# fundamentalvision/BEVFormer

Hardware: NVIDIA H100
Metric: BEV queries/sec (bevformer_base 200x200x256, 6 cams) fwd+bwd (higher is better)
Workload: dtype bf16

## Files before the change

bevformer_b200/_lib.py:

```python
from __future__ import annotations

import ctypes
import os
import threading

from . import build as _build

_lock = threading.Lock()
_lib = None

c_void_p, c_int, c_int64 = ctypes.c_void_p, ctypes.c_int, ctypes.c_int64

SIGNATURES = {
    "bevf_version": (c_int, []),
    "bevf_last_error": (ctypes.c_char_p, []),
    "bevf_launch_count": (c_int64, []),
    "bevf_msda_forward": (c_int, [c_void_p, c_int, c_void_p, c_void_p, c_void_p, c_void_p,
                                  c_void_p, c_int] + [c_int] * 7 + [c_void_p]),
    "bevf_msda_backward": (c_int, [c_void_p, c_int, c_void_p, c_void_p, c_void_p, c_void_p,
                                   c_void_p, c_int, c_void_p, c_void_p, c_void_p] + [c_int] * 7
                           + [c_void_p]),
    "bevf_msda_rows_forward": (c_int, [c_void_p, c_int, c_void_p, c_void_p, c_void_p, c_void_p,
                                       c_void_p, c_int, c_void_p] + [c_int] * 7 + [c_void_p]),
    "bevf_msda_rows_backward": (c_int, [c_void_p, c_int, c_void_p, c_void_p, c_void_p, c_void_p,
                                        c_void_p, c_int, c_void_p, c_void_p, c_void_p, c_void_p]
                                + [c_int] * 7 + [c_void_p]),
    "bevf_msda_rows_backward_ordered": (c_int, [c_void_p, c_int, c_void_p, c_void_p, c_void_p, c_void_p,
                                                c_void_p, c_int, c_void_p, c_void_p, c_void_p, c_void_p,
                                                c_void_p] + [c_int] * 7 + [c_void_p]),
    "bevf_msda_set_backward_mode": (c_int, [c_int]),
    "bevf_abs_max": (c_int, [c_void_p, c_int, c_int64, c_void_p, c_void_p]),
    "bevf_msda_rows_backward_f16acc": (c_int, [c_void_p, c_int, c_void_p, c_void_p, c_void_p, c_void_p, c_void_p, c_int,
                                               c_void_p, c_void_p, c_void_p, c_void_p, c_void_p, c_void_p] + [c_int] * 7
                                       + [c_void_p]),
    "bevf_gv16_unscale": (c_int, [c_void_p, c_void_p, c_void_p, c_int64, c_void_p]),
    "bevf_msda_rows_backward_mixed": (c_int, [c_void_p, c_int, c_void_p, c_void_p, c_void_p, c_void_p, c_void_p, c_void_p,
                                              c_int, c_void_p, c_void_p, c_void_p, c_int, c_void_p, c_void_p, c_void_p,
                                              c_void_p] + [c_int] * 7 + [c_void_p]),
    "bevf_gv_merge": (c_int, [c_void_p, c_void_p, c_void_p, c_void_p, c_int, c_int, c_int, c_int, c_void_p]),
    "bevf_msda_fx_frac_bits": (c_int, [c_int64, c_int, c_int]),
    "bevf_msda_backward_fx": (c_int, [c_void_p, c_int, c_void_p, c_void_p, c_void_p, c_void_p, c_void_p, c_int,
                                      c_void_p, c_void_p, c_int, c_void_p, c_void_p] + [c_int] * 7 + [c_void_p]),
    "bevf_msda_rows_backward_fx": (c_int, [c_void_p, c_int, c_void_p, c_void_p, c_void_p, c_void_p, c_void_p, c_int,
                                           c_void_p, c_void_p, c_int, c_void_p, c_void_p, c_void_p] + [c_int] * 7
                                   + [c_void_p]),
    "bevf_msda_fx_convert": (c_int, [c_void_p, c_void_p, c_int, c_void_p, c_int, c_int, c_int64, c_void_p]),
    "bevf_msda_rows_backward_dense": (c_int, [c_void_p, c_int, c_void_p, c_void_p, c_void_p, c_void_p, c_void_p,
                                              c_void_p, c_int, c_void_p, c_void_p, c_void_p, c_void_p, c_void_p]
                                      + [c_int] * 7 + [c_void_p]),
    "bevf_msda_set_dense_backward": (c_int, [c_int]),
    "bevf_msda_get_dense_backward": (c_int, []),
    "bevf_msda_dense_plan": (c_int, [c_void_p, c_int, c_int, c_int, c_void_p, c_int, c_void_p]),
    "bevf_sca_plan_workspace_ints": (c_int64, [c_int, c_int]),
    "bevf_sca_plan_build": (c_int, [c_void_p] * 10 + [c_int] * 5 + [c_void_p]),
    "bevf_msda_rows_forward_staged": (c_int, [c_void_p, c_int, c_void_p, c_void_p, c_void_p, c_void_p, c_void_p,
                                              c_void_p, c_int, c_void_p] + [c_int] * 7 + [c_void_p]),
    "bevf_sca_prep_forward": (c_int, [c_void_p] * 7 + [c_int] * 8 + [c_void_p]),
    "bevf_sca_prep_backward": (c_int, [c_void_p] * 6 + [c_int] * 8 + [c_void_p]),
    "bevf_tsa_prep_forward": (c_int, [c_void_p] * 5 + [c_int] * 6 + [c_void_p]),
    "bevf_tsa_prep_backward": (c_int, [c_void_p] * 5 + [c_int] * 7 + [c_void_p]),
    "bevf_layernorm_forward": (c_int, [c_void_p] * 4 + [c_int] + [c_void_p] * 5
# ... 89 lines not shown
```

bevformer_b200/csrc/msda.cu:

```cuda
#include <cuda_fp16.h>

#include <cstdlib>
#include <cstring>
#include <type_traits>

#include "msda_common.cuh"

namespace bevf {

template <typename T, typename TO>
__global__ void __launch_bounds__(kThreads)
msda_fwd_d32(const T *__restrict__ value, const int64_t *__restrict__ level_hw,
             const int64_t *__restrict__ level_start, const float *__restrict__ loc,
             const float *__restrict__ attn, TO *__restrict__ out,
             const int *__restrict__ row_map, int S, int M, int Q, int L, int P, int magic,
             int iters, long long rows) {
    constexpr int VEC = Vec<T>::N, LANES = 32 / VEC, G = 32 / LANES;
    constexpr bool kHalf = std::is_same<T, bf16>::value;
    __shared__ LevelTab tab;
    load_level_tab(level_hw, level_start, L, M * 32, tab);

    const int lane = threadIdx.x & 31, warp = threadIdx.x >> 5;
    const int sub = lane % LANES, grp = lane / LANES;
    for (int it = 0; it < iters; ++it) {
    long long row = (((long long)blockIdx.x * (kThreads / 32) + warp) * iters + it) * G + grp;
    if (row - grp >= rows) break;
// ... 456 lines not shown

static std::atomic<int> g_bwd_mode{-1};
static int bwd_split_enabled() {
    int v = g_bwd_mode.load(std::memory_order_relaxed);
    if (v < 0) {
        const char *e = getenv("BEVF_MSDA_BWD");
        v = (e && e[0] == 's') ? 1 : 0;
        g_bwd_mode.store(v, std::memory_order_relaxed);
    }
    return v;
}
static unsigned splat_direct_mask() {
    static long v = -1;
    if (v < 0) {
        const char *e = getenv("BEVF_SPLAT_DIRECT");
        v = e ? strtol(e, nullptr, 0) : 0;
    }
    return (unsigned)v;
}

int dense_coarse_backward(const char *who, const int64_t *hw_dev, const int64_t *ls_dev, const int32_t *hw_host,
                          const float *loc, const float *attn, const void *grad_out, float *grad_value,
                          const int32_t *map_range, int NB, int S, int M, int L, int P, cudaStream_t st,
                          unsigned *handled, HostLevels *host_levels);

static cudaStream_t g_side_stream = nullptr;
constexpr int kSideEvents = 64;
static cudaEvent_t g_side_events[kSideEvents];
static std::atomic<unsigned> g_side_ev_next{0};

template <typename TG, int kM>
static int launch_splat_km(const char *who, const float *loc, const float *attn, const void *go, float *gv,
                           const int *row_map, const int *order, const int64_t *hw, const int64_t *ls,
                           int S, int M, int Q, int L, int P, long long pairs, unsigned level_mask,
                           cudaStream_t st) {
    static bool attr_done = false;
    if (!attr_done) {
        if (cudaFuncSetAttribute(msda_bwd_splat_d32<TG, kM>, cudaFuncAttributeMaxDynamicSharedMemorySize,
                                 (int)splat_smem_bytes(kSplatMaxHeads, sizeof(TG))) != cudaSuccess) {
            cudaGetLastError();
            return fail("%s: cannot reserve shared memory for the splat kernel", who);
        }
        attr_done = true;
    }
    const unsigned grid = (unsigned)((pairs + kSplatG - 1) / kSplatG);
    msda_bwd_splat_d32<TG, kM><<<grid, 32 * M, splat_smem_bytes(M, sizeof(TG)), st>>>(
        loc, attn, (const TG *)go, gv, row_map, order, hw, ls, S, M, Q, L, P, pairs, splat_direct_mask(),
// ... 60 lines not shown
        if constexpr (std::is_same<T, bf16>::value) {
            if (D != 32) return fail("%s: fp16 grad_value needs head_dim 32", who);
            constexpr int G = Vec<T>::N;
            const int iters = pick_iters(rows, G);
            const long long per_block = (long long)(kThreads / 32) * G * iters;
            const unsigned grid = (unsigned)((rows + per_block - 1) / per_block);
            msda_bwd_d32<T, TG, true, __half><<<grid, kThreads, 0, st>>>((const T *)value, hw, ls, loc, attn, (const TG *)go,
                                                                       reinterpret_cast<__half *>(gv), gl, ga, row_map, S, M,
                                                                       Q, L, P, (65536 + P - 1) / P, iters, rows, 0u, hl,
                                                                       mixed ? mixed->amax : nullptr);
            return check_launch(who);
        } else {
            return fail("%s: fp16 grad_value needs a bf16 value tensor", who);
        }
    }
    if (mixed && mixed->gv16) {
        if constexpr (std::is_same<T, bf16>::value) {
            if (D != 32) return fail("%s: mixed accumulation needs head_dim 32", who);
            constexpr int G = Vec<T>::N;
            const int iters = pick_iters(rows, G);
            const long long per_block = (long long)(kThreads / 32) * G * iters;
            const unsigned grid = (unsigned)((rows + per_block - 1) / per_block);
            msda_bwd_d32<T, TG, true><<<grid, kThreads, 0, st>>>((const T *)value, hw, ls, loc, attn, (const TG *)go, gv, gl, ga,
                                                               row_map, S, M, Q, L, P, (65536 + P - 1) / P, iters, rows, 0u,
                                                               hl, mixed->amax, mixed->gv16, mixed->mask, mixed->side_start,
                                                               mixed->S_side);
            return check_launch(who);
        } else {
            return fail("%s: mixed accumulation needs a bf16 value tensor", who);
        }
    }
    if (D == 32) {
        constexpr int G = Vec<T>::N;
        const int iters = pick_iters(rows, G);
        const long long per_block = (long long)(kThreads / 32) * G * iters;
        const unsigned grid = (unsigned)((rows + per_block - 1) / per_block);
        const int mode = done_levels ? 0 : bwd_split_enabled();
        if (mode != 0 && std::is_same<T, __half>::value)
            return fail("%s: the split / hybrid backward modes take fp32 or bf16 only (fp16 needs mode 0)", who);
        const bool can_split = M <= kSplatMaxHeads && S * (long long)M * 32 < (1ll << 31);
        if (mode == 1 && can_split) {
            if (int e = launch_splat<TG>(who, loc, attn, go, gv, row_map, order, hw, ls, S, M, Q, L, P,
                                         rows / M, 0xffffffffu, st))
                return e;
            msda_bwd_d32<T, TG, false><<<grid, kThreads, 0, st>>>((const T *)value, hw, ls, loc, attn,
                                                                  (const TG *)go, gv, gl, ga, row_map, S, M,
                                                                  Q, L, P, (65536 + P - 1) / P, iters, rows, 0u, hl);
        } else if (mode == 2 && can_split && L >= 2 && g_side_stream) {
// ... 107 lines not shown

extern "C" int bevf_msda_rows_forward(const void *value, int value_dtype, const int64_t *level_hw,
                                      const int64_t *level_start, const float *loc,
                                      const float *attn, void *out, int out_dtype,
                                      const int32_t *row_map, int B, int S, int M, int D, int R,
                                      int L, int P, void *stream) {
    if (!row_map && R > 0) return fail("%s: row_map is null", "bevf_msda_rows_forward");
    return msda_forward_impl("bevf_msda_rows_forward", value, value_dtype, level_hw, level_start,
                             loc, attn, out, out_dtype, row_map, B, S, M, D, R, L, P, stream);
}

extern "C" int bevf_msda_rows_backward(const void *value, int value_dtype, const int64_t *level_hw,
                                       const int64_t *level_start, const float *loc,
                                       const float *attn, const void *grad_out, int grad_out_dtype,
                                       float *grad_value, float *grad_loc, float *grad_attn,
                                       const int32_t *row_map, int B, int S, int M, int D, int R,
                                       int L, int P, void *stream) {
    if (!row_map && R > 0) return fail("%s: row_map is null", "bevf_msda_rows_backward");
    return msda_backward_impl("bevf_msda_rows_backward", value, value_dtype, level_hw, level_start,
                              loc, attn, grad_out, grad_out_dtype, grad_value, grad_loc, grad_attn,
                              row_map, nullptr, B, S, M, D, R, L, P, stream);
}

static std::atomic<int> g_dense_mode{-1};
static int dense_mode() {
    int v = g_dense_mode.load(std::memory_order_relaxed);
    if (v < 0) {
        const char *e = getenv("BEVF_MSDA_DENSE");
        v = e ? atoi(e) : 0;
        if (v < 0 || v > 1) v = 1;
        g_dense_mode.store(v, std::memory_order_relaxed);
    }
    return v;
}
static int ensure_side_stream(const char *who) {
    if (g_side_stream) return 0;
    if (cudaStreamCreateWithFlags(&g_side_stream, cudaStreamNonBlocking) != cudaSuccess) {
        cudaGetLastError();
        g_side_stream = nullptr;
        return fail("%s: cannot create the second stream", who);
    }
    for (int i = 0; i < kSideEvents; ++i) cudaEventCreateWithFlags(&g_side_events[i], cudaEventDisableTiming);
    return 0;
}

extern "C" int bevf_msda_set_dense_backward(int mode) {
    if (mode < 0 || mode > 2)
        return fail("%s: mode must be 0 (off), 1 (same stream) or 2 (second stream)", "bevf_msda_set_dense_backward");
    if (mode == 2)
        if (int e = ensure_side_stream("bevf_msda_set_dense_backward")) return e;
    g_dense_mode.store(mode, std::memory_order_relaxed);
    return 0;
}

extern "C" int bevf_msda_get_dense_backward(void) { return dense_mode(); }

extern "C" int bevf_msda_rows_backward_dense(const void *value, int value_dtype, const int64_t *level_hw,
                                             const int64_t *level_start, const int32_t *level_hw_host,
                                             const float *loc, const float *attn, const void *grad_out,
                                             int grad_out_dtype, float *grad_value, float *grad_loc,
                                             float *grad_attn, const int32_t *row_map, const int32_t *map_range,
                                             int B, int S, int M, int D, int R, int L, int P, void *stream) {
    const char *who = "bevf_msda_rows_backward_dense";
    if (!row_map && R > 0) return fail("%s: row_map is null", who);
    if (int e = check_dims(who, B, S, M, D, R, L, P)) return e;
    if (R == 0) return 0;
    if (!level_hw_host || !map_range || !level_hw || !level_start || !loc || !attn || !grad_out || !grad_value)
        return fail("%s: null pointer argument", who);
    cudaStream_t st = (cudaStream_t)stream;
    unsigned handled = 0;
    HostLevels hl;
    memset(&hl, 0, sizeof(hl));
    const int mode = dense_mode();
    cudaEvent_t join = nullptr;
    if (value_dtype == BEVF_DTYPE_F16 || grad_out_dtype == BEVF_DTYPE_F16)
        return fail("%s: fp32 or bf16 only (fp16 runs on bevf_msda_rows_backward)", who);
    if (mode != 0 && D == 32 && grad_out_dtype == BEVF_DTYPE_BF16 && aligned16(loc) && aligned16(attn) &&
        aligned16(grad_out) && aligned16(grad_value)) {
        cudaStream_t ds = st;
        if (mode == 2 && g_side_stream) {
            cudaEvent_t fork = g_side_events[g_side_ev_next.fetch_add(1) % kSideEvents];
            join = g_side_events[g_side_ev_next.fetch_add(1) % kSideEvents];
            cudaEventRecord(fork, st);
            cudaStreamWaitEvent(g_side_stream, fork, 0);
            ds = g_side_stream;
        }
        const int e = dense_coarse_backward(who, level_hw, level_start, level_hw_host, loc, attn, grad_out, grad_value,
                                            map_range, B, S, M, L, P, ds, &handled, &hl);
        if (join) cudaEventRecord(join, g_side_stream);
        if (e) {
            if (join) cudaStreamWaitEvent(st, join, 0);
            return e;
        }
    }
    const int e = msda_backward_impl(who, value, value_dtype, level_hw, level_start, loc, attn, grad_out,
                                     grad_out_dtype, grad_value, grad_loc, grad_attn, row_map, nullptr, B, S, M, D,
                                     R, L, P, stream, handled, &hl);
    if (join) cudaStreamWaitEvent(st, join, 0);
    return e;
}

extern "C" int bevf_msda_rows_backward_f16acc(const void *value, int value_dtype, const int64_t *level_hw,
                                              const int64_t *level_start, const float *loc, const float *attn,
                                              const void *grad_out, int grad_out_dtype, void *grad_value_f16,
                                              const uint32_t *amax_bits, float *grad_loc, float *grad_attn,
                                              const int32_t *row_map, const int32_t *group_order, int B, int S,
                                              int M, int D, int R, int L, int P, void *stream) {
    const char *who = "bevf_msda_rows_backward_f16acc";
    if (!row_map && R > 0) return fail("%s: row_map is null", who);
    if (!grad_value_f16 || !amax_bits) return fail("%s: null pointer argument", who);
    MixedGv mx;
    mx.amax = amax_bits;
    return msda_backward_impl(who, value, value_dtype, level_hw, level_start, loc, attn, grad_out, grad_out_dtype,
                              reinterpret_cast<float *>(grad_value_f16), grad_loc, grad_attn, row_map, group_order, B, S,
                              M, D, R, L, P, stream, 0u, nullptr, true, &mx);
}

extern "C" int bevf_msda_rows_backward_mixed(const void *value, int value_dtype, const int64_t *level_hw,
                                             const int64_t *level_start, const int32_t *level_hw_host,
                                             const float *loc, const float *attn, const void *grad_out,
                                             int grad_out_dtype, void *grad_value_fine_f16, float *grad_value_side,
                                             const uint32_t *amax_bits, int num_f16_levels, float *grad_loc,
                                             float *grad_attn, const int32_t *row_map, const int32_t *group_order,
                                             int B, int S, int M, int D, int R, int L, int P, void *stream) {
    const char *who = "bevf_msda_rows_backward_mixed";
    if (!row_map && R > 0) return fail("%s: row_map is null", who);
    if (!level_hw_host || !grad_value_fine_f16 || !grad_value_side || !amax_bits)
        return fail("%s: null pointer argument", who);
    if (L <= 1 || L > kMaxLevels || num_f16_levels < 1 || num_f16_levels >= L)
        return fail("%s: num_f16_levels must be in [1, L - 1]", who);
    if (value_dtype != BEVF_DTYPE_BF16 || D != 32) return fail("%s: needs a bf16 value tensor and head_dim 32", who);
    if (!aligned16(grad_value_fine_f16) || !aligned16(grad_value_side))
        return fail("%s: device pointers must be 16-byte aligned", who);
    HostLevels hl;
    memset(&hl, 0, sizeof(hl));
    long long start = 0;
    for (int l = 0; l < L; ++l) {
        const int h = level_hw_host[2 * l], w = level_hw_host[2 * l + 1];
        if (h <= 0 || w <= 0 || h >= 32768 || w >= 32768) return fail("%s: bad host level shape", who);
        hl.h[l] = h; hl.w[l] = w; hl.start[l] = (int)start;
        start += (long long)h * w;
    }
    if (start != S) return fail("%s: host level shapes do not add up to S (%lld vs %lld)", who, start, S);
    MixedGv mx;
    mx.amax = amax_bits;
    mx.gv16 = reinterpret_cast<__half *>(grad_value_fine_f16);
    mx.mask = (1u << num_f16_levels) - 1u;
    mx.side_start = hl.start[num_f16_levels];
    mx.S_side = S - mx.side_start;
    return msda_backward_impl(who, value, value_dtype, level_hw, level_start, loc, attn, grad_out, grad_out_dtype,
                              grad_value_side, grad_loc, grad_attn, row_map, group_order, B, S, M, D, R, L, P, stream, 0u,
                              &hl, false, &mx);
}

namespace bevf {
int fx_bounds_launch(const char *who, const float *attn, const void *grad_out, int grad_out_dtype,
                     const int32_t *row_map, long long qrows, int M, int D, int L, int P, uint32_t *bounds,
                     cudaStream_t st);

static int msda_backward_fx_impl(const char *who, const void *value, int value_dtype, const int64_t *level_hw,
                                 const int64_t *level_start, const float *loc, const float *attn, const void *grad_out,
                                 int grad_out_dtype, int64_t *grad_value_fx, uint32_t *bounds, int frac_bits,
                                 float *grad_loc, float *grad_attn, const int32_t *row_map, int B, int S, int M, int D,
                                 int Q, int L, int P, void *stream) {
    if (int e = check_dims(who, B, S, M, D, Q, L, P)) return e;
    const long long qrows = (row_map ? 1ll : (long long)B) * Q;
    if (qrows == 0) return 0;
    if (!bounds || !grad_value_fx || !attn || !grad_out) return fail("%s: null pointer argument", who);
    const int kmax = bevf_msda_fx_frac_bits(Q, L, P);
    if (frac_bits < 0 || frac_bits > kmax)
        return fail("%s: frac_bits must be in [0, %lld] for this launch (bevf_msda_fx_frac_bits)", who, kmax);
    cudaStream_t st = (cudaStream_t)stream;
    if (int e = fx_bounds_launch(who, attn, grad_out, grad_out_dtype, row_map, qrows, M, D, L, P, bounds, st)) return e;
    FxGv fx;
    fx.bounds = bounds;
// ... 57 lines not shown
```

bevformer_b200/csrc/msda_dense.cu:

```cuda
#include <cuda.h>

#include <cstdlib>
#include <cstring>
#include <mutex>

#include "msda_common.cuh"

namespace bevf {

constexpr int kDnK = 16;
constexpr int kDnMaxBins = 32;
constexpr int kDnBinLevels = 4;
constexpr int kDnTileBytes = 128 * kDnK * 2;
constexpr int kDnTransposeBytes = 16 * 144;

struct DenseBins {
    int nbins, L;
    int s0[kDnMaxBins], n[kDnMaxBins];
    int nlev[kDnMaxBins];
    int lev[kDnMaxBins][kDnBinLevels];
    HostLevels hl;
};

namespace dn {
// ... 60 lines not shown
    uint4 v;
    asm volatile("ld.global.nc.v4.u32 {%0, %1, %2, %3}, [%4];" : "=r"(v.x), "=r"(v.y), "=r"(v.z), "=r"(v.w) : "l"(p));
    return v;
}
__device__ __forceinline__ unsigned short lds16(uint32_t addr) {
    unsigned short h;
    asm volatile("ld.shared.u16 %0, [%1];" : "=h"(h) : "r"(addr) : "memory");
    return h;
}
__device__ __forceinline__ void sts16(uint32_t addr, unsigned short h) {
    asm volatile("st.shared.u16 [%0], %1;" ::"r"(addr), "h"(h) : "memory");
}
__device__ __forceinline__ unsigned short bf16_add(unsigned short old, float x) {
    const float v = __uint_as_float((uint32_t)old << 16) + x;
    return __bfloat16_as_ushort(__float2bfloat16_rn(v));
}
}

template <int kTiles, int P, int NT>
__global__ void __launch_bounds__(128 * NT + 256, 1)
msda_bwd_dense_tc(const __grid_constant__ DenseBins bins, const int64_t *__restrict__ level_hw,
                  const int64_t *__restrict__ level_start, const float *__restrict__ loc,
                  const float *__restrict__ attn, const bf16 *__restrict__ grad_out,
                  float *__restrict__ grad_value, const int *__restrict__ map_range, int NB, int S, int M, int L,
                  int chunk_rows, int dbg) {
    static_assert(P == 4 || P == 8, "points per level: 4 or 8");
    static_assert(kTiles == 4, "accumulator tiles per bin: 2 per issuer warpgroup");
    static_assert(NT >= 1 && NT <= 3, "scatter teams");
    constexpr int kThreadsAll = 128 * NT + 256;
    constexpr int kSlabBytes = kTiles * kDnTileBytes;
    constexpr int kMine = kTiles / 2;
    constexpr int kColsPerWarp = 32 / P;
    constexpr int kWarpsPerLevel = kDnK / kColsPerWarp;
    constexpr int kLevelsPerPass = 4 / kWarpsPerLevel;
    constexpr int kMaxPass = kDnBinLevels / kLevelsPerPass;
    extern __shared__ __align__(1024) uint8_t smem_raw[];
    uint8_t *smem = reinterpret_cast<uint8_t *>((reinterpret_cast<uintptr_t>(smem_raw) + 1023) & ~uintptr_t(1023));
    uint8_t *slab = smem;
    uint8_t *gtile = smem + NT * kSlabBytes;
    float *tr = reinterpret_cast<float *>(gtile + NT * 4096);
    uint64_t *bar_full = reinterpret_cast<uint64_t *>(reinterpret_cast<uint8_t *>(tr) + 8 * kDnTransposeBytes);
    uint64_t *bar_empty = bar_full + NT;
    uint32_t *s_dirty = reinterpret_cast<uint32_t *>(bar_empty + NT);
    __shared__ int s_h[kMaxLevels], s_w[kMaxLevels], s_start[kMaxLevels];
    __shared__ int s_bad;

    const int tid = threadIdx.x, lane = tid & 31;
    const int team = tid >> 7, tt = tid & 127, tw = tt >> 5;
// ... 242 lines not shown
                float *trw = tr + (iw * 4 + w4) * (kDnTransposeBytes / 4);
                const int sub = lane & 7;
#pragma unroll
                for (int i = 0; i < kMine; ++i) {
                    const int tile = 2 * i + iw;
                    if (!((udirty >> tile) & 1u)) continue;
#pragma unroll
                    for (int h = 0; h < 2; ++h) {
#pragma unroll
                        for (int j = 0; j < 4; ++j)
#pragma unroll
                            for (int hh = 0; hh < 2; ++hh)
                                *reinterpret_cast<float2 *>(trw + (8 * hh + (lane >> 2)) * 36 + 8 * j + 2 * (lane & 3)) =
                                    make_float2(acc[i][h][4 * j + 2 * hh], acc[i][h][4 * j + 2 * hh + 1]);
                        __syncwarp();
#pragma unroll
                        for (int q = 0; q < 4; ++q) {
                            const int rr = 4 * q + (lane >> 3);
                            const int row = tile * 128 + h * 64 + w4 * 16 + rr;
                            const float4 v = *reinterpret_cast<const float4 *>(trw + rr * 36 + sub * 4);
                            const bool nz = ((__float_as_uint(v.x) | __float_as_uint(v.y) | __float_as_uint(v.z) |
                                              __float_as_uint(v.w)) & 0x7fffffffu) != 0u;
                            if (nz && row < nb) {
                                float *gp = grad_value + (((long long)b * S + s0 + row) * M + m) * 32 + sub * 4;
                                red_add_v4(gp, v.x, v.y, v.z, v.w);
                            }
                        }
                        __syncwarp();
                    }
                }
            }
            unit_bar();
        }
    }
}

}

namespace bevf {

static long dense_env(const char *name, long dflt) {
    const char *e = getenv(name);
    return e ? strtol(e, nullptr, 0) : dflt;
}

static int plan_dense_bins(const int32_t *hw_host, int L, long max_pix, int cap, DenseBins &bins, long long *total) {
    memset(&bins, 0, sizeof(bins));
    bins.L = L;
    long long start = 0;
    unsigned mask = 0;
    int open = -1;
    for (int l = 0; l < L; ++l) {
        const int h = hw_host[2 * l], w = hw_host[2 * l + 1];
        if (h <= 0 || w <= 0 || h >= 32768 || w >= 32768) return -1;
        const long long n = (long long)h * w;
        bins.hl.h[l] = h; bins.hl.w[l] = w; bins.hl.start[l] = (int)start;
        if (n <= max_pix) {
            if (n <= cap && open >= 0 && bins.n[open] + n <= cap && bins.nlev[open] < kDnBinLevels) {
                bins.lev[open][bins.nlev[open]++] = l;
                bins.n[open] += (int)n;
            } else {
                const int parts = (int)((n + cap - 1) / cap);
                if (bins.nbins + parts > kDnMaxBins) return -2;
                long long off = 0;
                for (int i = 0; i < parts; ++i) {
                    const int bi = bins.nbins++;
                    bins.s0[bi] = (int)(start + off);
                    bins.n[bi] = (int)((n - off) < cap ? (n - off) : cap);
                    bins.nlev[bi] = 1;
                    bins.lev[bi][0] = l;
                    off += bins.n[bi];
                }
                open = bins.nbins - 1;
            }
            mask |= 1u << l;
        } else {
            open = -1;
        }
        start += n;
    }
    *total = start;
    return (int)mask;
}

int dense_coarse_backward(const char *who, const int64_t *hw_dev, const int64_t *ls_dev, const int32_t *hw_host,
                          const float *loc, const float *attn, const void *grad_out, float *grad_value,
                          const int32_t *map_range, int NB, int S, int M, int L, int P, cudaStream_t st,
                          unsigned *handled, HostLevels *host_levels) {
    *handled = 0;
    static const long max_pix = dense_env("BEVF_DENSE_MAXPIX", 8192);
    static const long tiles = dense_env("BEVF_DENSE_TILES", 4);
    static const long chunk = dense_env("BEVF_DENSE_CHUNK", 512);
    if ((P != 4 && P != 8) || L > kMaxLevels || NB <= 0 || max_pix <= 0) return 0;
    if (tiles != 4) return fail("%s: BEVF_DENSE_TILES must be 4", who);
    if (chunk < kDnK || chunk % kDnK) return fail("%s: BEVF_DENSE_CHUNK must be a positive multiple of 16", who);
    const int cap = (int)tiles * 128;
    DenseBins bins;
    long long start = 0;
    const int pm = plan_dense_bins(hw_host, L, max_pix, cap, bins, &start);
    if (pm == -1) return fail("%s: bad host level shape", who);
    if (pm == -2) return 0;
    const unsigned mask = (unsigned)pm;
    if (start != S) return fail("%s: host level shapes do not add up to S (%lld vs %lld)", who, start, S);
    if (mask == 0) return 0;
    static int sms = 0;
    if (sms == 0) {
        int dev = 0;
        cudaGetDevice(&dev);
        cudaDeviceGetAttribute(&sms, cudaDevAttrMultiProcessorCount, dev);
    }
    static const long teams_env = dense_env("BEVF_DENSE_TEAMS", 0);
    const int teams = teams_env > 0 ? (int)teams_env : 2;
    const size_t smem = 1024 + (size_t)teams * ((size_t)tiles * kDnTileBytes + 4096) + 8 * kDnTransposeBytes + 256;
    static const long dbg = dense_env("BEVF_DENSE_DEBUG", 0);
    auto launch = [&](auto kern) -> int {
        static const void *configured[16];
        static int nconfigured = 0;
        static std::mutex mu;
        {
            std::lock_guard<std::mutex> lock(mu);
            bool seen = false;
            for (int i = 0; i < nconfigured; ++i) seen = seen || configured[i] == (const void *)kern;
            if (!seen) {
                if (cudaFuncSetAttribute(kern, cudaFuncAttributeMaxDynamicSharedMemorySize, (int)smem) != cudaSuccess) {
                    cudaGetLastError();
                    return fail("%s: cannot reserve shared memory for the dense backward", who);
                }
                if (nconfigured < 16) configured[nconfigured++] = (const void *)kern;
            }
        }
        kern<<<(unsigned)sms, 128 * teams + 256, smem, st>>>(bins, hw_dev, ls_dev, loc, attn, (const bf16 *)grad_out,
                                                           grad_value, map_range, NB, S, M, L, (int)chunk, (int)dbg);
        return check_launch(who);
    };
    int e;
    if (teams == 3) e = (P == 8) ? launch(msda_bwd_dense_tc<4, 8, 3>) : launch(msda_bwd_dense_tc<4, 4, 3>);
    else if (teams == 2) e = (P == 8) ? launch(msda_bwd_dense_tc<4, 8, 2>) : launch(msda_bwd_dense_tc<4, 4, 2>);
    else if (teams == 1) e = (P == 8) ? launch(msda_bwd_dense_tc<4, 8, 1>) : launch(msda_bwd_dense_tc<4, 4, 1>);
    else return fail("%s: BEVF_DENSE_TEAMS must be 1, 2 or 3", who);
    if (e) return e;
    *handled = mask;
    *host_levels = bins.hl;
    return 0;
}

}

extern "C" int bevf_msda_dense_plan(const int32_t *level_hw_host, int L, int max_pix, int tiles, int32_t *bins_out,
                                    int bins_cap, uint32_t *level_mask) {
    using namespace bevf;
    const char *who = "bevf_msda_dense_plan";
    if (!level_hw_host || !bins_out || !level_mask || L <= 0 || L > kMaxLevels || (tiles != 4 && tiles != 8 && tiles != 16))
        return -fail("%s: bad argument", who);
    DenseBins bins;
    long long total = 0;
// ... 13 lines not shown
```

bevformer_b200/ops.py:

```python
from __future__ import annotations

import os
import warnings

import torch
from torch.autograd.function import Function, once_differentiable

from . import _lib

F32, BF16, F16 = 0, 1, 2
_DT = {torch.float32: F32, torch.bfloat16: BF16, torch.float16: F16}
TC_DTYPES = (torch.bfloat16, torch.float16)


def deterministic() -> bool:
    return torch.are_deterministic_algorithms_enabled()


def alert_not_deterministic(name: str) -> None:
    if not torch.are_deterministic_algorithms_enabled():
        return
    msg = (f"{name} does not have a deterministic implementation, but you set "
           "'torch.use_deterministic_algorithms(True)'.")
    if torch.is_deterministic_algorithms_warn_only_enabled():
# ... 267 lines not shown
                                                 grad_output.data_ptr(), _DT[grad_output.dtype],
                                                 grad_value.data_ptr(), grad_loc.data_ptr(),
                                                 grad_attn.data_ptr(), row_map.data_ptr(), _ptr(group_order),
                                                 NB, S, M, D, R, L, P, _stream_ptr(value))
    _lib.check(st, lib)
    return grad_value, grad_loc, grad_attn


def gv_mode_for(rows_per_map: float, num_points: int, level_hw_host):
    if os.environ.get("BEVF_GV_ACC", "f16") != "f16" or not level_hw_host:
        return None
    cap = float(os.environ.get("BEVF_GV_MAXCONTRIB", "64"))
    shapes = [(int(h), int(w)) for h, w in level_hw_host]
    nfine = 0
    for h, w in shapes:
        if rows_per_map * num_points * 4.0 / (h * w) > cap:
            break
        nfine += 1
    if nfine == 0:
        return None
    return "f16" if nfine == len(shapes) else ("mixed", shapes, nfine)


class LazyGradValue:

    def __init__(self, shape, fine, side, amax):
        self.shape, self.fine, self.side, self.amax = tuple(shape), fine, side, amax
        self.tensors = tuple(t for t in (fine, side, amax) if t is not None)
        self.device = fine.device

    def materialize(self) -> torch.Tensor:
        nb, s, m, d = self.shape
        gv = torch.empty(self.shape, device=self.device, dtype=torch.bfloat16)
        lib = _lib.load()
        with torch.cuda.device(self.device):
            if self.side is None:
                st = lib.bevf_gv16_unscale(self.fine.data_ptr(), self.amax.data_ptr(), gv.data_ptr(), gv.numel(),
                                           _stream_ptr(gv))
            else:
                st = lib.bevf_gv_merge(self.fine.data_ptr(), self.side.data_ptr(), self.amax.data_ptr(), gv.data_ptr(),
                                       nb, s, self.fine.shape[1], m * d, _stream_ptr(gv))
        _lib.check(st, lib)
        return gv


class FixedPointGradValue(LazyGradValue):
# ... 79 lines not shown
    if value.dtype != torch.bfloat16 or value.shape[-1] != 32:
        raise RuntimeError("fp16-accumulated backward: value must be bfloat16 with head_dim 32")
    NB, S, M, D = value.shape
    R, _, L, P, _ = loc.shape
    ss, ls = _level_tensors(value, spatial_shapes, level_start_index)
    grad_output = grad_output.contiguous()
    grad_loc = torch.empty(loc.shape, device=value.device, dtype=torch.float32)
    grad_attn = torch.empty(attn.shape, device=value.device, dtype=torch.float32)
    lib = _lib.load()
    with torch.cuda.device(value.device), _timed("msda_rows_backward", value.device, (R, L)):
        amax = abs_max_bits(grad_output)
        gv16 = torch.zeros(value.shape, device=value.device, dtype=torch.float16)
        st = lib.bevf_msda_rows_backward_f16acc(value.data_ptr(), _DT[value.dtype], ss.data_ptr(), ls.data_ptr(),
                                                loc.data_ptr(), attn.data_ptr(), grad_output.data_ptr(),
                                                _DT[grad_output.dtype], gv16.data_ptr(), amax.data_ptr(),
                                                grad_loc.data_ptr(), grad_attn.data_ptr(), row_map.data_ptr(),
                                                _ptr(group_order), NB, S, M, D, R, L, P, _stream_ptr(value))
        _lib.check(st, lib)
    gv = LazyGradValue(value.shape, gv16, None, amax)
    return (gv if lazy else gv.materialize()), grad_loc, grad_attn


def msda_rows_backward_mixed(value, spatial_shapes, level_start_index, level_hw_host, num_f16_levels, loc, attn,
                             row_map, grad_output, group_order=None, lazy=False):
    import ctypes
    for t, n in ((value, "value"), (loc, "sampling_loc"), (attn, "attn_weight"), (row_map, "row_map"),
                 (grad_output, "grad_output")):
        _need_cuda(t, n)
    alert_not_deterministic("msda_rows_backward_mixed (grad_value summed with fp16 / fp32 atomics)")
    if value.dtype != torch.bfloat16 or value.shape[-1] != 32:
        raise RuntimeError("mixed-accumulation backward: value must be bfloat16 with head_dim 32")
    NB, S, M, D = value.shape
    R, _, L, P, _ = loc.shape
    if len(level_hw_host) != L or not (1 <= num_f16_levels < L):
        raise RuntimeError("mixed-accumulation backward: level_hw_host / num_f16_levels do not fit the pyramid")
    ss, ls = _level_tensors(value, spatial_shapes, level_start_index)
    s_fine = sum(int(h) * int(w) for h, w in level_hw_host[:num_f16_levels])
    grad_output = grad_output.contiguous()
    grad_loc = torch.empty(loc.shape, device=value.device, dtype=torch.float32)
    grad_attn = torch.empty(attn.shape, device=value.device, dtype=torch.float32)
    hw = (ctypes.c_int32 * (2 * L))(*[int(v) for hw_ in level_hw_host for v in hw_])
    lib = _lib.load()
    with torch.cuda.device(value.device), _timed("msda_rows_backward", value.device, (R, L)):
        amax = abs_max_bits(grad_output)
        fine = torch.zeros((NB, s_fine, M, D), device=value.device, dtype=torch.float16)
        side = torch.zeros((NB, S - s_fine, M, D), device=value.device, dtype=torch.float32)
        st = lib.bevf_msda_rows_backward_mixed(value.data_ptr(), _DT[value.dtype], ss.data_ptr(), ls.data_ptr(),
                                               ctypes.addressof(hw), loc.data_ptr(), attn.data_ptr(),
                                               grad_output.data_ptr(), _DT[grad_output.dtype], fine.data_ptr(),
                                               side.data_ptr(), amax.data_ptr(), int(num_f16_levels),
                                               grad_loc.data_ptr(), grad_attn.data_ptr(), row_map.data_ptr(),
                                               _ptr(group_order), NB, S, M, D, R, L, P, _stream_ptr(value))
        _lib.check(st, lib)
    gv = LazyGradValue(value.shape, fine, side, amax)
    return (gv if lazy else gv.materialize()), grad_loc, grad_attn


AUX_STREAM: dict = {}


def aux_stream(device):
    return AUX_STREAM.get(torch.device(device))


class SamplerRows(Function):

    @staticmethod
    def forward(ctx, value, loc, attn, row_map, spatial_shapes, level_start_index, group_order=None,
                staged=None, gv_mode=None):
        half = value.dtype == torch.float16
        if (staged is not None and not half and value.shape[-1] == 32
                and os.environ.get("BEVF_MSDA_FWD", "plain") == "staged"):
            out = msda_rows_forward_staged(value, spatial_shapes, level_start_index, staged[0], loc, attn,
                                           staged[1])
        else:
# ... 12 lines not shown
            ev.record(main)
            aux.wait_event(ev)
            with torch.cuda.stream(aux):
                gv0 = torch.zeros(value.shape, device=value.device, dtype=torch.float32)
                done = torch.cuda.Event()
                done.record(aux)
            gv0.record_stream(main)
            ctx.gv_zero = (gv0, done)
        return out

    @staticmethod
    @once_differentiable
    def backward(ctx, grad_out):
        value, loc, attn, row_map, ss, ls = ctx.saved_tensors
        if deterministic():
            gv, gl, ga = msda_backward_fx(value, ss, ls, loc, attn, grad_out.contiguous(), row_map)
            if ctx.value_early is not None and ctx.value_early(gv):
                return None, gl, ga, None, None, None, None, None, None
            return gv.materialize(), gl, ga, None, None, None, None, None, None
        gv0 = None
        if ctx.gv_zero is not None:
            gv0, done = ctx.gv_zero
            torch.cuda.current_stream(value.device).wait_event(done)
        dense_on = ctx.dense is not None and _lib.load().bevf_msda_get_dense_backward() != 0
        if ctx.gv_mode is not None and gv0 is None and grad_out.dtype == torch.bfloat16 and not dense_on:
            if ctx.gv_mode == "f16":
                gv, gl, ga = msda_rows_backward_f16acc(value, ss, ls, loc, attn, row_map, grad_out, ctx.group_order,
                                                       lazy=True)
            else:
                _, hw_host, nfine = ctx.gv_mode
                if sum(h * w for h, w in hw_host) != value.shape[1]:
                    gv, gl, ga = msda_rows_backward(value, ss, ls, loc, attn, row_map, grad_out.contiguous(), None,
                                                    group_order=ctx.group_order)
                    if ctx.value_early is not None and ctx.value_early(gv):
                        return None, gl, ga, None, None, None, None, None, None
                    return gv.to(value.dtype), gl, ga, None, None, None, None, None, None
                gv, gl, ga = msda_rows_backward_mixed(value, ss, ls, hw_host, nfine, loc, attn, row_map, grad_out,
                                                      ctx.group_order, lazy=True)
            if ctx.value_early is not None and ctx.value_early(gv):
                return None, gl, ga, None, None, None, None, None, None
            return gv.materialize(), gl, ga, None, None, None, None, None, None
        gv, gl, ga = msda_rows_backward(value, ss, ls, loc, attn, row_map, grad_out.contiguous(), gv0,
                                        group_order=ctx.group_order, dense=ctx.dense)
        if ctx.value_early is not None and ctx.value_early(gv):
            return None, gl, ga, None, None, None, None, None, None
        return gv.to(value.dtype), gl, ga, None, None, None, None, None, None


def sca_prep_forward(raw, ref_cam, pair_q, pair_cam, level_hw, B, Nq, M, L, P):
    _need_cuda(raw, "raw")
    R, D, ncam = pair_q.numel(), ref_cam.shape[3], ref_cam.shape[0]
    loc = torch.empty((B * R, M, L, P, 2), device=raw.device, dtype=torch.float32)
    attn = torch.empty((B * R, M, L, P), device=raw.device, dtype=torch.float32)
    lib = _lib.load()
    with torch.cuda.device(raw.device):
        st = lib.bevf_sca_prep_forward(raw.data_ptr(), ref_cam.data_ptr(), pair_q.data_ptr(),
                                       pair_cam.data_ptr(), level_hw.data_ptr(), loc.data_ptr(),
                                       attn.data_ptr(), B, Nq, R, M, L, P, D, ncam, _stream_ptr(raw))
    _lib.check(st, lib)
    return loc, attn

# ... 506 lines not shown
```

include/bevformer_b200.h:

```cpp
#ifndef BEVFORMER_B200_H_
#define BEVFORMER_B200_H_

#include <stdint.h>

#ifdef __cplusplus
extern "C" {
#endif

#define BEVF_ABI_VERSION 1

#if defined(__GNUC__)
#define BEVF_API __attribute__((visibility("default")))
#else
#define BEVF_API
#endif

enum bevf_dtype { BEVF_DTYPE_F32 = 0, BEVF_DTYPE_BF16 = 1, BEVF_DTYPE_F16 = 2 };

BEVF_API int bevf_version(void);

BEVF_API const char *bevf_last_error(void);

BEVF_API int64_t bevf_launch_count(void);

// ... 22 lines not shown
BEVF_API int bevf_msda_rows_backward_ordered(const void *value, int value_dtype, const int64_t *level_hw,
                                             const int64_t *level_start, const float *loc,
                                             const float *attn, const void *grad_out,
                                             int grad_out_dtype, float *grad_value, float *grad_loc,
                                             float *grad_attn, const int32_t *row_map,
                                             const int32_t *group_order, int B, int S, int M, int D,
                                             int R, int L, int P, void *stream);

BEVF_API int bevf_abs_max(const void *x, int dtype, int64_t n, uint32_t *amax_bits, void *stream);
BEVF_API int bevf_msda_rows_backward_f16acc(const void *value, int value_dtype, const int64_t *level_hw,
                                            const int64_t *level_start, const float *loc, const float *attn,
                                            const void *grad_out, int grad_out_dtype, void *grad_value_f16,
                                            const uint32_t *amax_bits, float *grad_loc, float *grad_attn,
                                            const int32_t *row_map, const int32_t *group_order, int B, int S,
                                            int M, int D, int R, int L, int P, void *stream);
BEVF_API int bevf_gv16_unscale(const void *gv16, const uint32_t *amax_bits, void *out_bf16, int64_t n, void *stream);
BEVF_API int bevf_msda_rows_backward_mixed(const void *value, int value_dtype, const int64_t *level_hw,
                                           const int64_t *level_start, const int32_t *level_hw_host,
                                           const float *loc, const float *attn, const void *grad_out,
                                           int grad_out_dtype, void *grad_value_fine_f16, float *grad_value_side,
                                           const uint32_t *amax_bits, int num_f16_levels, float *grad_loc,
                                           float *grad_attn, const int32_t *row_map, const int32_t *group_order,
                                           int B, int S, int M, int D, int R, int L, int P, void *stream);
BEVF_API int bevf_gv_merge(const void *fine_f16, const float *side_f32, const uint32_t *amax_bits, void *out_bf16,
                           int B, int S, int S_fine, int row_elems, void *stream);

BEVF_API int bevf_msda_fx_frac_bits(int64_t rows_per_map, int L, int P);
BEVF_API int bevf_msda_backward_fx(const void *value, int value_dtype, const int64_t *level_hw,
                                   const int64_t *level_start, const float *loc, const float *attn,
                                   const void *grad_out, int grad_out_dtype, int64_t *grad_value_fx, uint32_t *bounds,
                                   int frac_bits, float *grad_loc, float *grad_attn, int B, int S, int M, int D, int Q,
                                   int L, int P, void *stream);
BEVF_API int bevf_msda_rows_backward_fx(const void *value, int value_dtype, const int64_t *level_hw,
                                        const int64_t *level_start, const float *loc, const float *attn,
                                        const void *grad_out, int grad_out_dtype, int64_t *grad_value_fx,
                                        uint32_t *bounds, int frac_bits, float *grad_loc, float *grad_attn,
                                        const int32_t *row_map, int B, int S, int M, int D, int R, int L, int P,
                                        void *stream);
BEVF_API int bevf_msda_fx_convert(const int64_t *grad_value_fx, const uint32_t *bounds, int frac_bits, void *out,
                                  int out_dtype, int accumulate, int64_t n, void *stream);

BEVF_API int bevf_msda_rows_forward_staged(const void *value, int value_dtype, const int64_t *level_hw,
                                           const int64_t *level_start, const int32_t *level_hw_host,
                                           const float *loc, const float *attn, void *out, int out_dtype,
                                           const int32_t *map_range, int B, int S, int M, int D, int R,
                                           int L, int P, void *stream);
// ... 130 lines not shown
```

Measured before the change: 1.613 million.

## Combine dense tensor-core coarse-level backward with mixed-precision grad-value path

```diff
diff --git a/bevformer_b200/_lib.py b/bevformer_b200/_lib.py
--- a/bevformer_b200/_lib.py
+++ b/bevformer_b200/_lib.py
@@ -37,6 +37,9 @@
     "bevf_msda_rows_backward_mixed": (c_int, [c_void_p, c_int, c_void_p, c_void_p, c_void_p, c_void_p, c_void_p, c_void_p,
                                               c_int, c_void_p, c_void_p, c_void_p, c_int, c_void_p, c_void_p, c_void_p,
                                               c_void_p] + [c_int] * 7 + [c_void_p]),
+    "bevf_msda_rows_backward_mixed_dense": (c_int, [c_void_p, c_int, c_void_p, c_void_p, c_void_p, c_void_p, c_void_p,
+                                                    c_void_p, c_int, c_void_p, c_void_p, c_void_p, c_int, c_int,
+                                                    c_void_p, c_void_p, c_void_p, c_void_p] + [c_int] * 7 + [c_void_p]),
     "bevf_gv_merge": (c_int, [c_void_p, c_void_p, c_void_p, c_void_p, c_int, c_int, c_int, c_int, c_void_p]),
     "bevf_msda_fx_frac_bits": (c_int, [c_int64, c_int, c_int]),
     "bevf_msda_backward_fx": (c_int, [c_void_p, c_int, c_void_p, c_void_p, c_void_p, c_void_p, c_void_p, c_int,
diff --git a/bevformer_b200/csrc/msda.cu b/bevformer_b200/csrc/msda.cu
--- a/bevformer_b200/csrc/msda.cu
+++ b/bevformer_b200/csrc/msda.cu
@@ -2,6 +2,7 @@
 
 #include <cstdlib>
 #include <cstring>
+#include <mutex>
 #include <type_traits>
 
 #include "msda_common.cuh"
@@ -504,7 +505,8 @@
 int dense_coarse_backward(const char *who, const int64_t *hw_dev, const int64_t *ls_dev, const int32_t *hw_host,
                           const float *loc, const float *attn, const void *grad_out, float *grad_value,
                           const int32_t *map_range, int NB, int S, int M, int L, int P, cudaStream_t st,
-                          unsigned *handled, HostLevels *host_levels);
+                          unsigned *handled, HostLevels *host_levels, int first_level, unsigned need_mask,
+                          int gv_S, int gv_base);
 
 static cudaStream_t g_side_stream = nullptr;
 constexpr int kSideEvents = 64;
@@ -611,8 +613,8 @@
             const long long per_block = (long long)(kThreads / 32) * G * iters;
             const unsigned grid = (unsigned)((rows + per_block - 1) / per_block);
             msda_bwd_d32<T, TG, true><<<grid, kThreads, 0, st>>>((const T *)value, hw, ls, loc, attn, (const TG *)go, gv, gl, ga,
-                                                               row_map, S, M, Q, L, P, (65536 + P - 1) / P, iters, rows, 0u,
-                                                               hl, mixed->amax, mixed->gv16, mixed->mask, mixed->side_start,
+                                                               row_map, S, M, Q, L, P, (65536 + P - 1) / P, iters, rows,
+                                                               done_levels, hl, mixed->amax, mixed->gv16, mixed->mask, mixed->side_start,
                                                                mixed->S_side);
             return check_launch(who);
         } else {
@@ -766,38 +768,50 @@
                               row_map, nullptr, B, S, M, D, R, L, P, stream);
 }
 
-static std::atomic<int> g_dense_mode{-1};
-static int dense_mode() {
+constexpr int kDenseDefault = 2;
+static std::atomic<int> g_dense_mode{-2};
+static int dense_setting() {
     int v = g_dense_mode.load(std::memory_order_relaxed);
-    if (v < 0) {
+    if (v == -2) {
         const char *e = getenv("BEVF_MSDA_DENSE");
-        v = e ? atoi(e) : 0;
-        if (v < 0 || v > 1) v = 1;
+        v = -1;
+        if (e && e[0]) {
+            v = atoi(e);
+            if (v < 0 || v > 1) v = 1;
+        }
         g_dense_mode.store(v, std::memory_order_relaxed);
     }
     return v;
 }
+static int mixed_dense_mode() {
+    const int v = dense_setting();
+    return v < 0 ? kDenseDefault : v;
+}
 static int ensure_side_stream(const char *who) {
+    static std::mutex mu;
+    std::lock_guard<std::mutex> lock(mu);
     if (g_side_stream) return 0;
-    if (cudaStreamCreateWithFlags(&g_side_stream, cudaStreamNonBlocking) != cudaSuccess) {
+    cudaStream_t s = nullptr;
+    if (cudaStreamCreateWithFlags(&s, cudaStreamNonBlocking) != cudaSuccess) {
         cudaGetLastError();
-        g_side_stream = nullptr;
         return fail("%s: cannot create the second stream", who);
     }
     for (int i = 0; i < kSideEvents; ++i) cudaEventCreateWithFlags(&g_side_events[i], cudaEventDisableTiming);
+    g_side_stream = s;
     return 0;
 }
 
 extern "C" int bevf_msda_set_dense_backward(int mode) {
-    if (mode < 0 || mode > 2)
-        return fail("%s: mode must be 0 (off), 1 (same stream) or 2 (second stream)", "bevf_msda_set_dense_backward");
+    if (mode < -1 || mode > 2)
+        return fail("%s: mode must be -1 (library default), 0 (off), 1 (same stream) or 2 (second stream)",
+                    "bevf_msda_set_dense_backward");
     if (mode == 2)
         if (int e = ensure_side_stream("bevf_msda_set_dense_backward")) return e;
     g_dense_mode.store(mode, std::memory_order_relaxed);
     return 0;
 }
 
-extern "C" int bevf_msda_get_dense_backward(void) { return dense_mode(); }
+extern "C" int bevf_msda_get_dense_backward(void) { return mixed_dense_mode(); }
 
 extern "C" int bevf_msda_rows_backward_dense(const void *value, int value_dtype, const int64_t *level_hw,
                                              const int64_t *level_start, const int32_t *level_hw_host,
@@ -815,7 +829,7 @@
     unsigned handled = 0;
     HostLevels hl;
     memset(&hl, 0, sizeof(hl));
-    const int mode = dense_mode();
+    const int mode = dense_setting() < 0 ? 0 : dense_setting();
     cudaEvent_t join = nullptr;
     if (value_dtype == BEVF_DTYPE_F16 || grad_out_dtype == BEVF_DTYPE_F16)
         return fail("%s: fp32 or bf16 only (fp16 runs on bevf_msda_rows_backward)", who);
@@ -830,7 +844,7 @@
             ds = g_side_stream;
         }
         const int e = dense_coarse_backward(who, level_hw, level_start, level_hw_host, loc, attn, grad_out, grad_value,
-                                            map_range, B, S, M, L, P, ds, &handled, &hl);
+                                            map_range, B, S, M, L, P, ds, &handled, &hl, 0, 0u, S, 0);
         if (join) cudaEventRecord(join, g_side_stream);
         if (e) {
             if (join) cudaStreamWaitEvent(st, join, 0);
@@ -860,19 +874,20 @@
                               M, D, R, L, P, stream, 0u, nullptr, true, &mx);
 }
 
-extern "C" int bevf_msda_rows_backward_mixed(const void *value, int value_dtype, const int64_t *level_hw,
-                                             const int64_t *level_start, const int32_t *level_hw_host,
-                                             const float *loc, const float *attn, const void *grad_out,
-                                             int grad_out_dtype, void *grad_value_fine_f16, float *grad_value_side,
-                                             const uint32_t *amax_bits, int num_f16_levels, float *grad_loc,
-                                             float *grad_attn, const int32_t *row_map, const int32_t *group_order,
-                                             int B, int S, int M, int D, int R, int L, int P, void *stream) {
-    const char *who = "bevf_msda_rows_backward_mixed";
+static int rows_backward_mixed_impl(const char *who, const void *value, int value_dtype, const int64_t *level_hw,
+                                    const int64_t *level_start, const int32_t *level_hw_host, const float *loc,
+                                    const float *attn, const void *grad_out, int grad_out_dtype,
+                                    void *grad_value_fine_f16, float *grad_value_side, const uint32_t *amax_bits,
+                                    int num_f16_levels, int first_dense_level, float *grad_loc, float *grad_attn,
+                                    const int32_t *row_map, const int32_t *group_order, const int32_t *map_range,
+                                    int B, int S, int M, int D, int R, int L, int P, void *stream) {
     if (!row_map && R > 0) return fail("%s: row_map is null", who);
     if (!level_hw_host || !grad_value_fine_f16 || !grad_value_side || !amax_bits)
         return fail("%s: null pointer argument", who);
     if (L <= 1 || L > kMaxLevels || num_f16_levels < 1 || num_f16_levels >= L)
         return fail("%s: num_f16_levels must be in [1, L - 1]", who);
+    if (map_range && (first_dense_level < num_f16_levels || first_dense_level >= L))
+        return fail("%s: first_dense_level must be in [num_f16_levels, L - 1]", who);
     if (value_dtype != BEVF_DTYPE_BF16 || D != 32) return fail("%s: needs a bf16 value tensor and head_dim 32", who);
     if (!aligned16(grad_value_fine_f16) || !aligned16(grad_value_side))
         return fail("%s: device pointers must be 16-byte aligned", who);
@@ -892,9 +907,70 @@
     mx.mask = (1u << num_f16_levels) - 1u;
     mx.side_start = hl.start[num_f16_levels];
     mx.S_side = S - mx.side_start;
-    return msda_backward_impl(who, value, value_dtype, level_hw, level_start, loc, attn, grad_out, grad_out_dtype,
-                              grad_value_side, grad_loc, grad_attn, row_map, group_order, B, S, M, D, R, L, P, stream, 0u,
-                              &hl, false, &mx);
+    cudaStream_t st = (cudaStream_t)stream;
+    unsigned dense_levels = 0;
+    cudaEvent_t join = nullptr;
+    const int mode = map_range ? mixed_dense_mode() : 0;
+    if (mode != 0 && R > 0 && grad_out_dtype == BEVF_DTYPE_BF16 && aligned16(loc) && aligned16(attn) &&
+        aligned16(grad_out)) {
+        cudaStream_t ds = st;
+        if (mode == 2 && !g_side_stream) {
+            cudaStreamCaptureStatus cs = cudaStreamCaptureStatusActive;
+            if (cudaStreamIsCapturing(st, &cs) != cudaSuccess) cudaGetLastError();
+            else if (cs == cudaStreamCaptureStatusNone && ensure_side_stream(who) != 0) cudaGetLastError();
+        }
+        if (mode == 2 && g_side_stream) {
+            cudaEvent_t fork = g_side_events[g_side_ev_next.fetch_add(1) % kSideEvents];
+            join = g_side_events[g_side_ev_next.fetch_add(1) % kSideEvents];
+            cudaEventRecord(fork, st);
+            cudaStreamWaitEvent(g_side_stream, fork, 0);
+            ds = g_side_stream;
+        }
+        const unsigned suffix = ((1u << L) - 1u) & ~((1u << first_dense_level) - 1u);
+        HostLevels dhl;
+        const int e = dense_coarse_backward(who, level_hw, level_start, level_hw_host, loc, attn, grad_out,
+                                            grad_value_side, map_range, B, S, M, L, P, ds, &dense_levels, &dhl,
+                                            first_dense_level, suffix, mx.S_side, mx.side_start);
+        if (join) cudaEventRecord(join, g_side_stream);
+        if (e) {
+            if (join) cudaStreamWaitEvent(st, join, 0);
+            return e;
+        }
+    }
+    const int e = msda_backward_impl(who, value, value_dtype, level_hw, level_start, loc, attn, grad_out, grad_out_dtype,
+                                     grad_value_side, grad_loc, grad_attn, row_map, group_order, B, S, M, D, R, L, P,
+                                     stream, dense_levels, &hl, false, &mx);
+    if (join) cudaStreamWaitEvent(st, join, 0);
+    return e;
+}
+
+extern "C" int bevf_msda_rows_backward_mixed(const void *value, int value_dtype, const int64_t *level_hw,
+                                             const int64_t *level_start, const int32_t *level_hw_host,
+                                             const float *loc, const float *attn, const void *grad_out,
+                                             int grad_out_dtype, void *grad_value_fine_f16, float *grad_value_side,
+                                             const uint32_t *amax_bits, int num_f16_levels, float *grad_loc,
+                                             float *grad_attn, const int32_t *row_map, const int32_t *group_order,
+                                             int B, int S, int M, int D, int R, int L, int P, void *stream) {
+    return rows_backward_mixed_impl("bevf_msda_rows_backward_mixed", value, value_dtype, level_hw, level_start,
+                                    level_hw_host, loc, attn, grad_out, grad_out_dtype, grad_value_fine_f16,
+                                    grad_value_side, amax_bits, num_f16_levels, L, grad_loc, grad_attn, row_map,
+                                    group_order, nullptr, B, S, M, D, R, L, P, stream);
+}
+
+extern "C" int bevf_msda_rows_backward_mixed_dense(const void *value, int value_dtype, const int64_t *level_hw,
+                                                   const int64_t *level_start, const int32_t *level_hw_host,
+                                                   const float *loc, const float *attn, const void *grad_out,
+                                                   int grad_out_dtype, void *grad_value_fine_f16,
+                                                   float *grad_value_side, const uint32_t *amax_bits,
+                                                   int num_f16_levels, int first_dense_level, float *grad_loc,
+                                                   float *grad_attn, const int32_t *row_map, const int32_t *map_range,
+                                                   int B, int S, int M, int D, int R, int L, int P, void *stream) {
+    const char *who = "bevf_msda_rows_backward_mixed_dense";
+    if (!map_range) return fail("%s: null pointer argument", who);
+    return rows_backward_mixed_impl(who, value, value_dtype, level_hw, level_start, level_hw_host, loc, attn, grad_out,
+                                    grad_out_dtype, grad_value_fine_f16, grad_value_side, amax_bits, num_f16_levels,
+                                    first_dense_level, grad_loc, grad_attn, row_map, nullptr, map_range, B, S, M, D, R,
+                                    L, P, stream);
 }
 
 namespace bevf {
diff --git a/bevformer_b200/csrc/msda_dense.cu b/bevformer_b200/csrc/msda_dense.cu
--- a/bevformer_b200/csrc/msda_dense.cu
+++ b/bevformer_b200/csrc/msda_dense.cu
@@ -106,8 +106,8 @@
 msda_bwd_dense_tc(const __grid_constant__ DenseBins bins, const int64_t *__restrict__ level_hw,
                   const int64_t *__restrict__ level_start, const float *__restrict__ loc,
                   const float *__restrict__ attn, const bf16 *__restrict__ grad_out,
-                  float *__restrict__ grad_value, const int *__restrict__ map_range, int NB, int S, int M, int L,
-                  int chunk_rows, int dbg) {
+                  float *__restrict__ grad_value, const int *__restrict__ map_range, int NB, int gv_S, int gv_base,
+                  int M, int L, int chunk_rows, int dbg) {
     static_assert(P == 4 || P == 8, "points per level: 4 or 8");
     static_assert(kTiles == 4, "accumulator tiles per bin: 2 per issuer warpgroup");
     static_assert(NT >= 1 && NT <= 3, "scatter teams");
@@ -396,7 +396,7 @@
                             const bool nz = ((__float_as_uint(v.x) | __float_as_uint(v.y) | __float_as_uint(v.z) |
                                               __float_as_uint(v.w)) & 0x7fffffffu) != 0u;
                             if (nz && row < nb) {
-                                float *gp = grad_value + (((long long)b * S + s0 + row) * M + m) * 32 + sub * 4;
+                                float *gp = grad_value + (((long long)b * gv_S + s0 - gv_base + row) * M + m) * 32 + sub * 4;
                                 red_add_v4(gp, v.x, v.y, v.z, v.w);
                             }
                         }
@@ -418,7 +418,8 @@
     return e ? strtol(e, nullptr, 0) : dflt;
 }
 
-static int plan_dense_bins(const int32_t *hw_host, int L, long max_pix, int cap, DenseBins &bins, long long *total) {
+static int plan_dense_bins(const int32_t *hw_host, int L, long max_pix, int cap, DenseBins &bins, long long *total,
+                           int first = 0) {
     memset(&bins, 0, sizeof(bins));
     bins.L = L;
     long long start = 0;
@@ -429,7 +430,7 @@
         if (h <= 0 || w <= 0 || h >= 32768 || w >= 32768) return -1;
         const long long n = (long long)h * w;
         bins.hl.h[l] = h; bins.hl.w[l] = w; bins.hl.start[l] = (int)start;
-        if (n <= max_pix) {
+        if (l >= first && n <= max_pix) {
             if (n <= cap && open >= 0 && bins.n[open] + n <= cap && bins.nlev[open] < kDnBinLevels) {
                 bins.lev[open][bins.nlev[open]++] = l;
                 bins.n[open] += (int)n;
@@ -460,7 +461,8 @@
 int dense_coarse_backward(const char *who, const int64_t *hw_dev, const int64_t *ls_dev, const int32_t *hw_host,
                           const float *loc, const float *attn, const void *grad_out, float *grad_value,
                           const int32_t *map_range, int NB, int S, int M, int L, int P, cudaStream_t st,
-                          unsigned *handled, HostLevels *host_levels) {
+                          unsigned *handled, HostLevels *host_levels, int first_level, unsigned need_mask,
+                          int gv_S, int gv_base) {
     *handled = 0;
     static const long max_pix = dense_env("BEVF_DENSE_MAXPIX", 8192);
     static const long tiles = dense_env("BEVF_DENSE_TILES", 4);
@@ -471,12 +473,12 @@
     const int cap = (int)tiles * 128;
     DenseBins bins;
     long long start = 0;
-    const int pm = plan_dense_bins(hw_host, L, max_pix, cap, bins, &start);
+    const int pm = plan_dense_bins(hw_host, L, max_pix, cap, bins, &start, first_level);
     if (pm == -1) return fail("%s: bad host level shape", who);
     if (pm == -2) return 0;
     const unsigned mask = (unsigned)pm;
     if (start != S) return fail("%s: host level shapes do not add up to S (%lld vs %lld)", who, start, S);
-    if (mask == 0) return 0;
+    if (mask == 0 || (need_mask != 0 && mask != need_mask)) return 0;
     static int sms = 0;
     if (sms == 0) {
         int dev = 0;
@@ -484,7 +486,7 @@
         cudaDeviceGetAttribute(&sms, cudaDevAttrMultiProcessorCount, dev);
     }
     static const long teams_env = dense_env("BEVF_DENSE_TEAMS", 0);
-    const int teams = teams_env > 0 ? (int)teams_env : 2;
+    const int teams = teams_env > 0 ? (int)teams_env : 3;
     const size_t smem = 1024 + (size_t)teams * ((size_t)tiles * kDnTileBytes + 4096) + 8 * kDnTransposeBytes + 256;
     static const long dbg = dense_env("BEVF_DENSE_DEBUG", 0);
     auto launch = [&](auto kern) -> int {
@@ -504,7 +506,8 @@
             }
         }
         kern<<<(unsigned)sms, 128 * teams + 256, smem, st>>>(bins, hw_dev, ls_dev, loc, attn, (const bf16 *)grad_out,
-                                                           grad_value, map_range, NB, S, M, L, (int)chunk, (int)dbg);
+                                                           grad_value, map_range, NB, gv_S, gv_base, M, L, (int)chunk,
+                                                           (int)dbg);
         return check_launch(who);
     };
     int e;
diff --git a/bevformer_b200/ops.py b/bevformer_b200/ops.py
--- a/bevformer_b200/ops.py
+++ b/bevformer_b200/ops.py
@@ -313,6 +313,17 @@
     return "f16" if nfine == len(shapes) else ("mixed", shapes, nfine)
 
 
+def dense_levels_for(rows_per_map: float, num_points: int, level_hw_host):
+    shapes = [(int(h), int(w)) for h, w in level_hw_host]
+    first = None
+    for l in range(len(shapes) - 1, -1, -1):
+        h, w = shapes[l]
+        if rows_per_map * num_points * 4.0 / (h * w) <= 256:
+            break
+        first = l
+    return first
+
+
 class LazyGradValue:
 
     def __init__(self, shape, fine, side, amax):
@@ -438,7 +449,8 @@
 
 
 def msda_rows_backward_mixed(value, spatial_shapes, level_start_index, level_hw_host, num_f16_levels, loc, attn,
-                             row_map, grad_output, group_order=None, lazy=False):
+                             row_map, grad_output, group_order=None, lazy=False, map_range=None,
+                             first_dense_level=None):
     import ctypes
     for t, n in ((value, "value"), (loc, "sampling_loc"), (attn, "attn_weight"), (row_map, "row_map"),
                  (grad_output, "grad_output")):
@@ -450,6 +462,10 @@
     R, _, L, P, _ = loc.shape
     if len(level_hw_host) != L or not (1 <= num_f16_levels < L):
         raise RuntimeError("mixed-accumulation backward: level_hw_host / num_f16_levels do not fit the pyramid")
+    if map_range is not None:
+        _need_cuda(map_range, "map_range")
+        if group_order is not None or map_range.numel() != 2 * NB or map_range.dtype != torch.int32:
+            raise RuntimeError("mixed-accumulation backward: map_range must be (B, 2) int32, without group_order")
     ss, ls = _level_tensors(value, spatial_shapes, level_start_index)
     s_fine = sum(int(h) * int(w) for h, w in level_hw_host[:num_f16_levels])
     grad_output = grad_output.contiguous()
@@ -461,12 +477,17 @@
         amax = abs_max_bits(grad_output)
         fine = torch.zeros((NB, s_fine, M, D), device=value.device, dtype=torch.float16)
         side = torch.zeros((NB, S - s_fine, M, D), device=value.device, dtype=torch.float32)
-        st = lib.bevf_msda_rows_backward_mixed(value.data_ptr(), _DT[value.dtype], ss.data_ptr(), ls.data_ptr(),
-                                               ctypes.addressof(hw), loc.data_ptr(), attn.data_ptr(),
-                                               grad_output.data_ptr(), _DT[grad_output.dtype], fine.data_ptr(),
-                                               side.data_ptr(), amax.data_ptr(), int(num_f16_levels),
-                                               grad_loc.data_ptr(), grad_attn.data_ptr(), row_map.data_ptr(),
-                                               _ptr(group_order), NB, S, M, D, R, L, P, _stream_ptr(value))
+        args = (value.data_ptr(), _DT[value.dtype], ss.data_ptr(), ls.data_ptr(), ctypes.addressof(hw), loc.data_ptr(),
+                attn.data_ptr(), grad_output.data_ptr(), _DT[grad_output.dtype], fine.data_ptr(), side.data_ptr(),
+                amax.data_ptr(), int(num_f16_levels))
+        tail = (grad_loc.data_ptr(), grad_attn.data_ptr(), row_map.data_ptr())
+        if map_range is None:
+            st = lib.bevf_msda_rows_backward_mixed(*args, *tail, _ptr(group_order), NB, S, M, D, R, L, P,
+                                                   _stream_ptr(value))
+        else:
+            kd = num_f16_levels if first_dense_level is None else int(first_dense_level)
+            st = lib.bevf_msda_rows_backward_mixed_dense(*args, kd, *tail, map_range.data_ptr(), NB, S, M, D, R, L, P,
+                                                         _stream_ptr(value))
         _lib.check(st, lib)
     gv = LazyGradValue(value.shape, fine, side, amax)
     return (gv if lazy else gv.materialize()), grad_loc, grad_attn
@@ -525,8 +546,7 @@
         if ctx.gv_zero is not None:
             gv0, done = ctx.gv_zero
             torch.cuda.current_stream(value.device).wait_event(done)
-        dense_on = ctx.dense is not None and _lib.load().bevf_msda_get_dense_backward() != 0
-        if ctx.gv_mode is not None and gv0 is None and grad_out.dtype == torch.bfloat16 and not dense_on:
+        if ctx.gv_mode is not None and gv0 is None and grad_out.dtype == torch.bfloat16:
             if ctx.gv_mode == "f16":
                 gv, gl, ga = msda_rows_backward_f16acc(value, ss, ls, loc, attn, row_map, grad_out, ctx.group_order,
                                                        lazy=True)
@@ -538,8 +558,16 @@
                     if ctx.value_early is not None and ctx.value_early(gv):
                         return None, gl, ga, None, None, None, None, None, None
                     return gv.to(value.dtype), gl, ga, None, None, None, None, None, None
-                gv, gl, ga = msda_rows_backward_mixed(value, ss, ls, hw_host, nfine, loc, attn, row_map, grad_out,
-                                                      ctx.group_order, lazy=True)
+                kd = None
+                if ctx.dense is not None and ctx.group_order is None and _lib.load().bevf_msda_get_dense_backward():
+                    kd = dense_levels_for(row_map.numel() / max(1, value.shape[0]), loc.shape[3], hw_host)
+                if kd is not None:
+                    gv, gl, ga = msda_rows_backward_mixed(value, ss, ls, hw_host, nfine, loc, attn, row_map, grad_out,
+                                                          lazy=True, map_range=ctx.dense[1],
+                                                          first_dense_level=max(kd, nfine))
+                else:
+                    gv, gl, ga = msda_rows_backward_mixed(value, ss, ls, hw_host, nfine, loc, attn, row_map, grad_out,
+                                                          ctx.group_order, lazy=True)
             if ctx.value_early is not None and ctx.value_early(gv):
                 return None, gl, ga, None, None, None, None, None, None
             return gv.materialize(), gl, ga, None, None, None, None, None, None
diff --git a/include/bevformer_b200.h b/include/bevformer_b200.h
--- a/include/bevformer_b200.h
+++ b/include/bevformer_b200.h
@@ -68,6 +68,14 @@
                                            const uint32_t *amax_bits, int num_f16_levels, float *grad_loc,
                                            float *grad_attn, const int32_t *row_map, const int32_t *group_order,
                                            int B, int S, int M, int D, int R, int L, int P, void *stream);
+BEVF_API int bevf_msda_rows_backward_mixed_dense(const void *value, int value_dtype, const int64_t *level_hw,
+                                                 const int64_t *level_start, const int32_t *level_hw_host,
+                                                 const float *loc, const float *attn, const void *grad_out,
+                                                 int grad_out_dtype, void *grad_value_fine_f16, float *grad_value_side,
+                                                 const uint32_t *amax_bits, int num_f16_levels, int first_dense_level,
+                                                 float *grad_loc, float *grad_attn, const int32_t *row_map,
+                                                 const int32_t *map_range,
+                                                 int B, int S, int M, int D, int R, int L, int P, void *stream);
 BEVF_API int bevf_gv_merge(const void *fine_f16, const float *side_f32, const uint32_t *amax_bits, void *out_bf16,
                            int B, int S, int S_fine, int row_elems, void *stream);
 
```

Result: faster. 1.698 million, median of 6 (+5.2%).
